# 1pathplanningzzj/pointnet_refine

Measured on AMD Instinct MI355X. Metric: lane segments/sec (fwd+bwd) at B=4096,N=1024; HBM GB/s vs roofline, higher is better.
Workload: dtype f32 (large GEMMs: 2xfp16-split MFMA, 3 products, fp32 accumulate); 1 GPU; LineRefineNet training step (fwd + deep-supervision L1 + bwd + Adam), B=4096/GPU, N=1024, M=32, C=4; global_batch=4096, points=1024, parallelism=dp1, decoder_chunk=4096

## Files before the change

### include/pointnet_refine_hip.h

```cpp
#ifndef POINTNET_REFINE_HIP_H
#define POINTNET_REFINE_HIP_H

#include <stddef.h>
#include <stdint.h>

#ifdef __cplusplus
extern "C" {
#endif

#define PRH_OK 0
#define PRH_ERR_ARG (-1)
#define PRH_ERR_WORKSPACE (-2)
#define PRH_ERR_HIP (-3)

#define PRH_MAX_LAYERS 8

typedef struct {
  const float* w;
  const float* b;
  const float* gamma;
  const float* beta;
  float* running_mean;
  float* running_var;
  int64_t* num_batches_tracked;
// ... 25 lines not shown
} prh_encoder_grads;

typedef struct {
  float* z_cat;
  float* z_fus;
  float* gate;
  float* bn_scale;
  float* bn_shift;
  float* bn_mean;
  float* bn_rstd;
  int32_t* argmax;
  float* op_amax;
} prh_encoder_saved;

size_t prh_encoder_workspace_bytes(int B, int N, int in_channel, int out_dim, int backward);

int prh_encoder_forward(const prh_encoder_params* prm, const float* ctx, int B, int N,
                        int training, float momentum, float eps,
                        float* fused, float* gfeat, const prh_encoder_saved* saved,
                        void* workspace, size_t workspace_bytes, int device, void* stream);

int prh_encoder_backward(const prh_encoder_params* prm, const float* ctx, int B, int N,
                         int training, float* d_fused, const float* d_gfeat, int d_fused_scratch,
                         const prh_encoder_saved* saved, const prh_encoder_grads* grads,
                         float* d_ctx, void* workspace, size_t workspace_bytes, int device,
                         void* stream);

typedef struct {
  uint16_t* z_cat;
  uint16_t* z_fus;
// ... 276 lines not shown
```

### pointnet_refine_amd/_lib.py

```python
from __future__ import annotations

import ctypes as C
import os
import subprocess
import threading

_HERE = os.path.dirname(os.path.abspath(__file__))
_ROOT = os.path.dirname(_HERE)
LIB_PATH = os.environ.get("PRH_LIB_PATH") or os.path.join(_HERE, "libpointnet_refine_hip.so")
_CSRC = os.path.join(_HERE, "csrc")
_SOURCES = [os.path.join(_CSRC, "prh_lib.hip")] + (sorted(
    os.path.join(_CSRC, f) for f in os.listdir(_CSRC) if f.endswith((".hpp", ".h", ".hip")) and f != "prh_lib.hip")
    if os.path.isdir(_CSRC) else [])
_HEADER = os.path.join(_ROOT, "include", "pointnet_refine_hip.h")

PRH_MAX_LAYERS = 8


class BnLayer(C.Structure):
    _fields_ = [("w", C.c_void_p), ("b", C.c_void_p), ("gamma", C.c_void_p), ("beta", C.c_void_p),
                ("running_mean", C.c_void_p), ("running_var", C.c_void_p),
                ("num_batches_tracked", C.c_void_p), ("cin", C.c_int), ("cout", C.c_int)]


# ... 13 lines not shown


class EncoderSaved(C.Structure):
    _fields_ = [("z_cat", C.c_void_p), ("z_fus", C.c_void_p), ("gate", C.c_void_p),
                ("bn_scale", C.c_void_p), ("bn_shift", C.c_void_p), ("bn_mean", C.c_void_p),
                ("bn_rstd", C.c_void_p), ("argmax", C.c_void_p), ("op_amax", C.c_void_p)]


class EncoderSavedBf16(C.Structure):
    _fields_ = [("z_cat", C.c_void_p), ("z_fus", C.c_void_p), ("gate", C.c_void_p),
                ("bn_scale", C.c_void_p), ("bn_shift", C.c_void_p), ("bn_mean", C.c_void_p),
                ("bn_rstd", C.c_void_p), ("argmax", C.c_void_p)]


EXPORTS = [
    "prh_encoder_workspace_bytes", "prh_encoder_forward", "prh_encoder_backward",
    "prh_encoder_bf16_workspace_bytes", "prh_encoder_forward_bf16", "prh_encoder_backward_bf16",
    "prh_linear_bf16_workspace_bytes", "prh_linear_forward_bf16", "prh_linear_backward_bf16",
    "prh_linear_forward_out16", "prh_linear_backward_dy16", "prh_attn_forward_kv16", "prh_attn_backward_kv16",
    "prh_encoder_fused_image_bytes", "prh_encoder_fused_prepare", "prh_encoder_fused_workspace_bytes",
    "prh_encoder_fused_forward",
    "prh_linear_forward_workspace_bytes", "prh_linear_forward", "prh_linear_forward_ex",
    "prh_linear_forward_full", "prh_operand_absmax_workspace_bytes", "prh_operand_absmax",
    "prh_linear_uses_operand_maxima", "prh_linear_backward_full", "prh_pos_hidden_forward", "prh_pos_hidden_backward_workspace_bytes",
    "prh_pos_hidden_backward", "prh_linear_small_forward", "prh_linear_small_backward_workspace_bytes",
    "prh_linear_small_backward",
    "prh_linear_backward_workspace_bytes", "prh_linear_backward", "prh_linear_backward_ex",
    "prh_mlp_stack_workspace_bytes", "prh_mlp_stack_forward", "prh_mlp_stack_backward",
    "prh_test_gemm_nt", "prh_test_gemm_tn_workspace_bytes", "prh_test_gemm_tn",
    "prh_test_gemm_tn_side_workspace_bytes", "prh_test_gemm_tn_side", "prh_test_xcc_map",
    "prh_profile_enable", "prh_profile_count", "prh_profile_reset", "prh_profile_read",
# ... 35 lines not shown
    hipcc = os.environ.get("HIPCC", "/opt/rocm/bin/hipcc")
    cmd = [hipcc, "--offload-arch=gfx950", "-O3", "-std=c++17", "-shared", "-fPIC",
           "-o", LIB_PATH, _SOURCES[0]]
    if verbose:
        print(" ".join(cmd))
    subprocess.run(cmd, check=True)
    return LIB_PATH


def _bind(lib):
    vp, i, f, sz, lg = C.c_void_p, C.c_int, C.c_float, C.c_size_t, C.c_long
    lib.prh_last_error.restype = C.c_char_p
    lib.prh_version.restype = C.c_char_p
    lib.prh_encoder_workspace_bytes.restype = sz
    lib.prh_encoder_workspace_bytes.argtypes = [i, i, i, i, i]
    lib.prh_encoder_forward.restype = i
    lib.prh_encoder_forward.argtypes = [C.POINTER(EncoderParams), vp, i, i, i, f, f, vp, vp,
                                        C.POINTER(EncoderSaved), vp, sz, i, vp]
    lib.prh_encoder_backward.restype = i
    lib.prh_encoder_backward.argtypes = [C.POINTER(EncoderParams), vp, i, i, i, vp, vp, i,
                                         C.POINTER(EncoderSaved), C.POINTER(EncoderGrads), vp, vp,
                                         sz, i, vp]
    lib.prh_encoder_bf16_workspace_bytes.restype = sz
    lib.prh_encoder_bf16_workspace_bytes.argtypes = [i, i, i, i, i]
    lib.prh_encoder_forward_bf16.restype = i
    lib.prh_encoder_forward_bf16.argtypes = [C.POINTER(EncoderParams), vp, i, i, i, f, f, vp, vp,
                                             C.POINTER(EncoderSavedBf16), vp, sz, i, vp]
    lib.prh_encoder_backward_bf16.restype = i
    lib.prh_encoder_backward_bf16.argtypes = [C.POINTER(EncoderParams), vp, i, i, i, vp, vp,
                                              C.POINTER(EncoderSavedBf16), C.POINTER(EncoderGrads), vp, vp,
# ... 229 lines not shown
```

### pointnet_refine_amd/csrc/prh_gemm_h2.hpp

```cpp
#pragma once
#include "prh_gemm_s3.hpp"

namespace prh {

constexpr int H2_BK = 32;
constexpr int H2_PLANE = 256 * H2_BK * 2;
constexpr int H2_OPER = 2 * H2_PLANE;
constexpr int H2_STAGE = 2 * H2_OPER;
constexpr int H2_LDS = 2 * H2_STAGE;

__device__ __forceinline__ int h2_off(int row, int k) {
  return row * 64 + ((((k >> 3) ^ (-(row >> 2))) & 3) << 4) + ((k & 7) << 1);
}

inline size_t h2_weight_bytes(int N, int K) {
  return S3_WHDR + (size_t)((N + 255) / 256) * ((K + H2_BK - 1) / H2_BK) * H2_OPER;
}

__global__ __launch_bounds__(256) void prep_weights_h2_kernel(const float* __restrict__ W, int N,
                                                              int K, long ldw, char* __restrict__ out,
                                                              const float* __restrict__ amax) {
  const int KT = (K + H2_BK - 1) / H2_BK;
  const int NT_ = (N + 255) / 256;
  const long total = (long)NT_ * 256 * KT * 4;
// ... 584 lines not shown
    __syncthreads();
    if (tid < 64) {
      float4 s = red[tid];
#pragma unroll
      for (int g = 1; g < 8; ++g) {
        const float4 t = red[tid + 64 * g];
        s.x += t.x; s.y += t.y; s.z += t.z; s.w += t.w;
      }
      const float inv = 1.f / sA;
      float* o = p.colsum + (size_t)split * p.Mo + m0 + c4;
      if (m0 + c4 + 3 < p.Mo) { o[0] = s.x * inv; o[1] = s.y * inv; o[2] = s.z * inv; o[3] = s.w * inv; }
    }
  }
}

}
```

### pointnet_refine_amd/csrc/prh_kernels.hpp

```cpp
#pragma once
#include <hip/hip_runtime.h>
#include <stdint.h>

namespace prh {

constexpr int BN_SLICES = 32;

__global__ __launch_bounds__(256) void bn_stage1_kernel(const float* __restrict__ ws_a,
                                                        const float* __restrict__ ws_b, int R,
                                                        long ld, int N, int tile_rows, int P,
                                                        int forward, double* __restrict__ out) {
  __shared__ double red[3][8][33];
  const int c = threadIdx.x & 31, g = threadIdx.x >> 5;
  const int col = blockIdx.x * 32 + c, sl = blockIdx.y;
  const int per = (R + BN_SLICES - 1) / BN_SLICES;
  const int r0 = sl * per, r1 = (r0 + per < R) ? r0 + per : R;
  const bool ok = col < N;
  double a = 0.0, b = 0.0, n = 0.0;
  if (ok)
    for (int i = r0 + g; i < r1; i += 8) {
      a += (double)ws_a[(size_t)i * ld + col];
      if (forward) {
        int ni = P - i * tile_rows;
        ni = ni > tile_rows ? tile_rows : (ni < 0 ? 0 : ni);
// ... 210 lines not shown
  int ix = 0;
  for (int t = 0; t < tiles_per_seg; ++t) {
    const size_t o = ((size_t)b * tiles_per_seg + t) * C + col;
    const float v = pmax[o];
    if (v > mx) { mx = v; ix = t * 128 + pidx[o]; }
    sum += psum[o];
  }
  gfeat[(size_t)b * 2 * C + col] = mx;
  gfeat[(size_t)b * 2 * C + C + col] = sum / (float)N;
  if (argmax != nullptr) argmax[(size_t)b * C + col] = ix;
}

__global__ __launch_bounds__(256) void combine_bwd_kernel(
    const float* dF, const float* __restrict__ d_gfeat, const int32_t* __restrict__ argmax,
    const float* __restrict__ zf, float* gate, const float* __restrict__ s,
    const float* __restrict__ t, int P, int N, int C, float* dy_out, float* ws_a, float* ws_b) {
  __shared__ float r1[4][64], r2[4][64];
  const int c = threadIdx.x & 63, g = threadIdx.x >> 6;
  const int col = blockIdx.y * 64 + c;
  const int row0 = blockIdx.x * 64 + g * 16;
  float s1 = 0.f, s2 = 0.f;
  if (col < C) {
    const float sc = s[col], sh = t[col];
    for (int i = 0; i < 16; ++i) {
      const int row = row0 + i;
      if (row >= P) break;
      const size_t off = (size_t)row * C + col;
      float d = dF != nullptr ? dF[off] : 0.f;
      if (d_gfeat != nullptr) {
        const int b = row / N, n = row - b * N;
        d += d_gfeat[(size_t)b * 2 * C + C + col] / (float)N;
        if (argmax[(size_t)b * C + col] == n) d += d_gfeat[(size_t)b * 2 * C + col];
      }
      const float z = zf[off], m = gate[off];
      const float pre = fmaf(z, sc, sh);
      const float r = fmaxf(pre, 0.f);
      const float sig = 2.f * m - 1.f;
      const float dy = pre > 0.f ? d * m : 0.f;
      gate[off] = d * r * 0.5f * sig * (1.f - sig);
      dy_out[off] = dy;
      s1 += dy;
      s2 = fmaf(dy, z, s2);
    }
  }
  r1[g][c] = s1; r2[g][c] = s2;
  __syncthreads();
  if (g == 0 && col < C) {
    for (int j = 1; j < 4; ++j) { s1 += r1[j][c]; s2 += r2[j][c]; }
    ws_a[(size_t)blockIdx.x * C + col] = s1;
    ws_b[(size_t)blockIdx.x * C + col] = s2;
  }
}

__global__ __launch_bounds__(256) void bn_apply_kernel(const float* __restrict__ z, long ldz,
                                                       const float* __restrict__ s,
                                                       const float* __restrict__ t, int P, int C,
                                                       int relu, float* y, long ldy) {
  const int col = blockIdx.y * 64 + (threadIdx.x & 63);
  const int row0 = blockIdx.x * 64 + (threadIdx.x >> 6) * 16;
  if (col >= C) return;
  const float sc = s[col], sh = t[col];
// ... 555 lines not shown
```

### pointnet_refine_amd/csrc/prh_lib.hip

```cpp
#include "../../include/pointnet_refine_hip.h"

#include <hip/hip_runtime.h>
#include <stdarg.h>
#include <stdio.h>
#include <string.h>

#include <mutex>
#include <vector>

#include <stdlib.h>

#include "prh_gemm.hpp"
#include "prh_attn.hpp"
#include "prh_attn16.hpp"
#include "prh_gemm_s3.hpp"
#include "prh_gemm_h2.hpp"
#include "prh_b16.hpp"
#include "prh_small.hpp"
#include "prh_attnfold.hpp"
#include "prh_fused.hpp"
#include "prh_context.hpp"
#include "prh_metrics.hpp"
#include "prh_drive.hpp"
#include "prh_match.hpp"
// ... 315 lines not shown
  if (n64 && (long)cdiv(p.M, 32) * cdiv(p.N, 64) >= 192) return launch_small_cfg<1, 2, 2, NN, EPI>(p, st);
  return launch_small_cfg<1, 1, 4, NN, EPI>(p, st);
}
constexpr int TN_SMALL_MAX_P = 16384;
inline bool small_tn_dims_ok(int P, int Mo, int Ni) {
  return P >= 64 && P <= TN_SMALL_MAX_P && (P & 63) == 0 && (Mo & 63) == 0 && (Ni & 63) == 0;
}
inline void small_tn_plan(int P, int Mo, int Ni, int& splits, int& rps) {
  const int tiles = (Mo / 64) * (Ni / 64), chunks = P / 64;
  int s = cdiv(512, tiles);
  s = s > chunks ? chunks : (s < 1 ? 1 : s);
  rps = cdiv(chunks, s) * 64;
  splits = cdiv(P, rps);
}

template <int PRO, int EPI>
int launch_nt(Cores c, NTParams& p, hipStream_t st, StatInfo* si = nullptr) {
  if (p.M <= 0 || p.N <= 0) return PRH_OK;
  if ((p.K & 3) || (PRO != PRO_GATE1 && (p.lda & 3)) || (p.ldw & 3) ||
      (PRO == PRO_BNBWD && (p.lda2 & 3)))
    return fail(PRH_ERR_ARG, "gemm_nt: K/lda/ldw must be multiples of 4 (K=%d lda=%ld ldw=%ld)",
                p.K, p.lda, p.ldw);
  if constexpr (PRO == PRO_NONE && EPI == EPI_BIAS) {
    if (c.mode == 4 && c.core == 2 && nt_b16_generic_ok(p)) return launch_nt_b16<PRO_NONE, EPI_BIAS, false, false>(p, st, si);
  }
  const bool want_pool = (p.flags & F_POOL) != 0;
  p.flags &= ~F_POOL;
  char nm[64];
  const double by = 4.0 * ((double)p.M * p.K * (PRO == PRO_BNBWD ? 2 : (PRO == PRO_GATE1 ? 0 : 1)) +
                           (double)p.M * p.N * (EPI == EPI_GATE ? 3 : (EPI == EPI_DGRAD ? 2 : 1)) +
                           (double)p.N * p.K);
  {
    if (p.wprep != nullptr && nt_use_s3(c, p.M, p.N, p.K) && p.lda <= 65536 && p.lda2 <= 65536 &&
        !(EPI == EPI_GATE && ((p.N | (int)p.ldc | (int)p.lde1 | (int)p.ldc2) & 3) != 0)) {
      const int KT = cdiv(p.K, S3_BK), NTl = cdiv(p.N, S3_BN);
      const long th = (long)NTl * 256 * KT * 2;
      float* hdr = reinterpret_cast<float*>(p.wprep);
      const char* img = p.wprep + S3_WHDR;
      if (c.core == 3) {
        if (p.amaxW == nullptr) {
          TRY_RC((measure_absmax<PRO_NONE>(p.W, p.ldw, nullptr, 0, nullptr, nullptr, nullptr, p.N, p.K, hdr, hdr + 64, st)));
          p.amaxW = hdr;
        }
        if (p.amaxA == nullptr) {
          TRY_RC((measure_absmax<PRO>(p.A, p.lda, p.A2, p.lda2, p.pa, p.pb, p.pc, p.M, p.K, hdr + 1, hdr + 64, st)));
          p.amaxA = hdr + 1;
// ... 81 lines not shown
    s = best;
  }
  const int minrows = pl.s3 ? 512 : 128;
  const int smax = cdiv(P, minrows) < 1 ? 1 : cdiv(P, minrows);
  if (s > smax) s = smax;
  if (s < 1) s = 1;
  int rps = cdiv(P, s);
  rps = cdiv(rps, bk) * bk;
  if (rps < bk) rps = bk;
  const int cap = (int)((2147483647L / (4L * (maxld < 4 ? 4 : maxld))) / bk * bk);
  if (pl.s3 && rps > cap) rps = cap;
  pl.splits = cdiv(P, rps) < 1 ? 1 : cdiv(P, rps);
  pl.rows_per_split = rps;
  return pl;
}
constexpr int TN_HDR = S3_HDR_FLOATS;
inline size_t tn_splits_bound(Cores cores, int P, int Mo, int Ni) {
  const size_t a = (size_t)tn_plan(cores, P, Mo, Ni, true).splits, b = (size_t)tn_plan(cores, P, Mo, Ni, false).splits;
  size_t c = (size_t)tn_plan(cores, P, Mo, Ni, true, 4).splits;
  if (small_tn_dims_ok(P, Mo, Ni)) {
    int ss, rr; small_tn_plan(P, Mo, Ni, ss, rr);
    if ((size_t)ss > c) c = (size_t)ss;
  }
  return a > b ? (a > c ? a : c) : (b > c ? b : c);
}
inline size_t tn_slab_floats(Cores c, int P, int Mo, int Ni) { return tn_splits_bound(c, P, Mo, Ni) * Mo * Ni + TN_HDR; }
inline size_t tn_colsum_floats(Cores c, int P, int Mo, int Ni) { return tn_splits_bound(c, P, Mo, Ni) * Mo; }

inline bool tn_side_ok(Cores c, const TNParams& p, const TNSide& s) {
  if (c.core != 3 || p.Mo <= 0 || p.Ni <= 0) return false;
  if (p.lda > TN_S3_MAX_LD || p.ldb > TN_S3_MAX_LD || p.lda2 > TN_S3_MAX_LD) return false;
  const TNPlan pl = tn_plan(c, p.P, p.Mo, p.Ni, true, p.lda > p.ldb ? p.lda : p.ldb);
  if (!pl.s3 || ((p.Mo | p.Ni | (int)p.lda | (int)p.ldb) & 3) != 0) return false;
  if ((long)pl.tiles_m * pl.tiles_n * pl.splits > ABSMAX_MAX_BLOCKS) return false;
// ... 1 lines not shown
         s.cols <= TR_SIDE_MAX_COLS && ((s.cols | (int)s.lddy | (int)s.ldz) & 3) == 0 && s.lddy <= 65536 &&
         s.ldz <= 65536 && al16(s.dy) && al16(s.z);
}

template <int PROA, int PROB>
int launch_tn(Cores c, TNParams& p, float* slab, float* colsum_slab, float* C, long ldc, float* colsum_out,
              hipStream_t st) {
  const bool side = p.side.dy != nullptr;
  if (side && !((PROA == PRO_NONE && (PROB == PRO_NONE || PROB == PRO_BNRELU)) && tn_side_ok(c, p, p.side)))
    return fail(PRH_ERR_ARG, "gemm_tn: this launch cannot carry a side job (Mo=%d Ni=%d P=%d)", p.Mo, p.Ni, p.P);
  if (p.Mo <= 0 || p.Ni <= 0) return PRH_OK;
  const bool ld_ok = p.lda <= TN_S3_MAX_LD && p.ldb <= TN_S3_MAX_LD && p.lda2 <= TN_S3_MAX_LD;
  long maxld = p.lda > p.ldb ? p.lda : p.ldb;
  if (PROA == PRO_BNBWD && p.lda2 > maxld) maxld = p.lda2;
  TNPlan pl = tn_plan(c, p.P, p.Mo, p.Ni, PROB != PRO_GATE1 && ld_ok, maxld);
  if (!pl.s3 && ((p.Mo & 3) || (p.Ni & 3) || (p.lda & 3) || (PROB != PRO_GATE1 && (p.ldb & 3))))
    return fail(PRH_ERR_ARG, "gemm_tn: Mo/Ni/lda/ldb must be multiples of 4 (Mo=%d Ni=%d)", p.Mo,
                p.Ni);
  p.tiles_m = pl.tiles_m; p.tiles_n = pl.tiles_n; p.splits = pl.splits;
  p.rows_per_split = pl.rows_per_split;
  p.slab = slab;
  p.colsum = colsum_out != nullptr ? colsum_slab : nullptr;
  const long blocks = (long)pl.tiles_m * pl.tiles_n * pl.splits;
  {
    char nm[64];
    const double by = 4.0 * ((double)p.P * p.Mo * (PROA == PRO_BNBWD ? 2 : 1) +
                             (double)p.P * (PROB == PRO_GATE1 ? 1 : p.Ni) + (double)p.Mo * p.Ni);
    bool done = false;
    if constexpr (PROB != PRO_GATE1) {
      if (pl.s3) {
        static const int attr_rc = allow_big_lds(gemm_tn_s3_kernel<PROA, PROB, 3>, gemm_tn_s3_kernel<PROA, PROB, 1>,
                                                 gemm_tn_s3_kernel<PROA, PROB, 2>);
        if (attr_rc != PRH_OK) return attr_rc;
        if (c.core == 3) {
          float* hdr = slab + (size_t)pl.splits * p.Mo * p.Ni;
          if (p.amaxA == nullptr) {
            TRY_RC((measure_absmax<PROA>(p.A, p.lda, p.A2, p.lda2, p.pa, p.pb, p.pc, p.P, p.Mo, hdr, hdr + 64, st)));
            p.amaxA = hdr;
          }
          if (p.amaxB == nullptr) {
            TRY_RC((measure_absmax<PROB>(p.B, p.ldb, nullptr, 0, p.qa, p.qb, nullptr, p.P, p.Ni, hdr + 1, hdr + 64, st)));
            p.amaxB = hdr + 1;
          }
// ... 381 lines not shown

struct LinearBwdWS { float* wT; float* slab; float* cslab; char* wprep; };
void linear_bwd_carve(Cores c, Arena& a, LinearBwdWS& w, int rows, int k, int n) {
  w.wprep = (char*)a.f(s3_weight_bytes(k, n) / sizeof(float) + 64);
  w.wT = a.f((size_t)k * n);
  w.slab = a.f(tn_slab_floats(c, rows, n, k));
  w.cslab = a.f(tn_colsum_floats(c, rows, n, k));
}
struct MlpWS { StackWS w; StackBwdScratch sc; float* dy_cat; };
void mlp_carve(Cores c, Arena& a, MlpWS& m, int P, const prh_bn_layer* ly, int L) {
  StackDims d = stack_dims(ly, L);
  stack_ws_carve(a, m.w, P, ly, L, max_cout(ly, L));
  stack_bwd_scratch_carve(c, a, m.sc, P, ly, L, 0, 0);
  m.dy_cat = a.f((size_t)P * d.off[L]);
}
struct EncWS { StackWS w; StackBwdScratch sc; float* fslab; float* fcslab; float* dy_cat; float* dyf; float* dU; float* gsum_a; float* gsum_b; };
void enc_carve(Cores c, Arena& a, EncWS& e, int P, const prh_bn_layer* conv, int cat, int od, int backward) {
  stack_ws_carve(a, e.w, P, conv, 5, cat > od ? cat : od, od, cat);
  if (!backward) return;
  stack_bwd_scratch_carve(c, a, e.sc, P, conv, 5, (size_t)od * cat, cat > od ? cat : od);
  const size_t fs = tn_slab_floats(c, P, od, cat), gs = tn_slab_floats(c, P, od, 64);
  const size_t fc = tn_colsum_floats(c, P, od, cat), gc = tn_colsum_floats(c, P, od, 64);
  e.fslab = a.f(fs > gs ? fs : gs);
  e.fcslab = a.f(fc > gc ? fc : gc);
  e.dy_cat = a.f((size_t)P * cat);
  e.dyf = backward == 2 ? nullptr : a.f((size_t)P * od);
  e.dU = a.f((size_t)P * 64);
  e.gsum_a = a.f(64);
  e.gsum_b = a.f(64);
}

typedef unsigned short u16;
struct Enc16WS {
  u16* xpad; float* w0pad; float* ws_a; float* ws_b; float* ws_c; double* stat2; char* wprep;
  float *ca, *cb, *cc, *wT, *slab, *cslab, *dU, *gsum_a, *gsum_b; u16 *dy_cat, *dyf;
  float* c1part;
};
constexpr int C1_WGRAD_BLOCKS = 1024;
inline bool conv_in_fp32_ok(int cin, int cout) { return cin <= 8 && cout == 64; }
inline int cin_pad8(int c) { return (c + 7) / 8 * 8; }
void enc16_carve(Arena& a, Enc16WS& e, int P, const int* ch , int cat, int od, bool backward) {
  const int c0p = cin_pad8(ch[0]);
  const int maxc = cat > od ? cat : od;
  e.xpad = (u16*)a.f(((size_t)P * c0p + 1) / 2);
// ... 397 lines not shown
  for (int l = 0; l < 5; ++l) c += prm->conv[l].cout;
  return c;
}

size_t prh_encoder_workspace_bytes(int B, int N, int in_channel, int out_dim, int backward) {
  const int P = B * N;
  prh_bn_layer ly[5];
  const int ch[6] = {in_channel, 64, 128, 256, 512, out_dim};
  for (int l = 0; l < 5; ++l) { ly[l].cin = ch[l]; ly[l].cout = ch[l + 1]; }
  const int cat = 64 + 128 + 256 + 512 + out_dim;
  Arena a; EncWS e;
  enc_carve(cores_of(gemm_mode()), a, e, P, ly, cat, out_dim, backward);
  return a.off + 256;
}

static int check_encoder(const prh_encoder_params* prm) {
  if (!prm) return fail(PRH_ERR_ARG, "encoder: null params");
  if (prm->in_channel < 4) return fail(PRH_ERR_ARG, "encoder: expected input to have at least 4 channels (x,y,z,intensity), got %d", prm->in_channel);
  if (prm->conv[0].cin != prm->in_channel) return fail(PRH_ERR_ARG, "encoder: conv1.cin != in_channel");
  TRY(check_stack(prm->conv, 5));
  if (prm->conv[4].cout != prm->out_dim) return fail(PRH_ERR_ARG, "encoder: conv5.cout != out_dim");
  if (prm->fusion.cin != enc_cat(prm) || prm->fusion.cout != prm->out_dim)
    return fail(PRH_ERR_ARG, "encoder: fusion layer shape mismatch");
  if (prm->out_dim % 4) return fail(PRH_ERR_ARG, "encoder: out_dim must be a multiple of 4");
  if (!prm->fusion.w || !prm->fusion.b || !prm->fusion.gamma || !prm->fusion.beta ||
      !prm->fusion.running_mean || !prm->fusion.running_var || !prm->gate_w1 || !prm->gate_b1 ||
      !prm->gate_w2 || !prm->gate_b2)
    return fail(PRH_ERR_ARG, "encoder: null parameter pointer");
  return PRH_OK;
}
// ... 87 lines not shown
    return fail(PRH_ERR_ARG, "encoder_backward: d_fused_scratch needs d_fused and no d_gfeat");
  enc_carve(c, a, ews, P, prm->conv, cat, od, d_fused_scratch ? 2 : 1);
  StackWS& w = ews.w;
  StackBwdScratch& sc = ews.sc;
  float *fslab = ews.fslab, *fcslab = ews.fcslab, *dy_cat = ews.dy_cat, *dU = ews.dU, *dyf = d_fused_scratch ? d_fused : ews.dyf;
  float *gsum_a = ews.gsum_a, *gsum_b = ews.gsum_b;
  if (!a.ok) return fail(PRH_ERR_WORKSPACE, "encoder_backward: workspace too small (%zu bytes)", workspace_bytes);
  StackDims d = stack_dims(prm->conv, 5);
  if (d.cin0p != d.cin0) {
    TRY(copy_cols(ctx, d.cin0, d.cin0, w.xpad, d.cin0p, d.cin0p, (size_t)P, st));
    TRY(copy_cols(prm->conv[0].w, d.cin0, d.cin0, w.w0pad, d.cin0p, d.cin0p, (size_t)prm->conv[0].cout, st));
  }

  hipLaunchKernelGGL(combine_bwd_kernel, dim3(cdiv(P, 64), cdiv(od, 64)), dim3(256), 0, st, d_fused,
                     d_gfeat, sv->argmax, sv->z_fus, sv->gate, sv->bn_scale + cat,
                     sv->bn_shift + cat, P, N, od, dyf, w.ws_a, w.ws_b);
  LAUNCH_CHECK();
  hipLaunchKernelGGL(bn_stage1_kernel, dim3(cdiv(od, 32), BN_SLICES), dim3(256), 0, st, w.ws_a, w.ws_b,
                     cdiv(P, 64), (long)od, od, 64, P, 0, w.stat2);
  LAUNCH_CHECK();
  hipLaunchKernelGGL(bn_bwd_finalize_kernel, dim3(cdiv(od, 128)), dim3(128), 0, st, w.stat2, P, od,
                     prm->fusion.gamma, sv->bn_mean + cat, sv->bn_rstd + cat,
                     training, sc.ca, sc.cb, sc.cc, gr->fusion.dgamma, gr->fusion.dbeta,
                     gr->fusion.db);
  LAUNCH_CHECK();
  float* dG = sv->gate;

  StatInfo si5;
  const float* dzf_amax = nullptr;
  const bool matf = dz_in_place(c, od, (long)od, (long)od);
  if (matf) {
    TRY(materialize_dz(dyf, (long)od, sv->z_fus, (long)od, sc.ca, sc.cb, sc.cc, P, od, sc.hdr[0], st));
// ... 25 lines not shown
    p.ws_a = w.ws_a; p.ws_b = w.ws_b;
    p.flags = F_MASK | F_STATS;
    if (matf) TRY((launch_nt<PRO_NONE, EPI_DGRAD>(c, p, st, &si5)));
    else TRY((launch_nt<PRO_BNBWD, EPI_DGRAD>(c, p, st, &si5)));
    si5.ld = cat; si5.off = d.off[4];
  }
  float* dx = d_ctx;
  TRY(stack_backward(c, prm->conv, 5, ctx, P, training, dy_cat, (long)cat, sv->z_cat, (long)cat,
                     sv->bn_scale, sv->bn_shift, sv->bn_mean, sv->bn_rstd, gr->conv, dx, w, sc, si5,
                     st, sv->op_amax, &hf));

  {
    TNParams t; memset(&t, 0, sizeof(t));
    t.A = dG; t.lda = od; t.B = ctx + 3; t.ldb = C; t.qa = prm->gate_w1; t.qb = prm->gate_b1;
    t.P = P; t.Mo = od; t.Ni = 64;
    TRY((launch_tn<PRO_NONE, PRO_GATE1>(c, t, fslab, fcslab, gr->d_gate_w2, 64L, gr->d_gate_b2, st)));
    TRY(transpose(prm->gate_w2, od, 64, sc.wT, st));
    NTParams p; memset(&p, 0, sizeof(p));
    p.A = dG; p.lda = od; p.W = sc.wT; p.ldw = od; p.M = P; p.N = 64; p.K = od;
    p.C = dU; p.ldc = 64; p.E1 = ctx + 3; p.lde1 = C; p.es = prm->gate_w1; p.et = prm->gate_b1;
    p.ws_a = w.ws_a; p.ws_b = w.ws_b;
    p.flags = F_MASK | F_STATS | F_E1_ROWVEC;
    StatInfo sig;
    TRY((launch_nt<PRO_NONE, EPI_DGRAD>(c, p, st, &sig)));
    hipLaunchKernelGGL(partials_reduce_kernel, dim3(2), dim3(1024), 0, st, w.ws_a, w.ws_b,
                       sig.count, 64, gr->d_gate_b1 ? gr->d_gate_b1 : gsum_a,
                       gr->d_gate_w1 ? gr->d_gate_w1 : gsum_b);
    LAUNCH_CHECK();
    if (d_ctx != nullptr) {
      hipLaunchKernelGGL(gate1_dctx_kernel, dim3(cdiv(P, 4)), dim3(256), 0, st, dU, P, 64,
                         prm->gate_w1, d_ctx, (long)C);
      LAUNCH_CHECK();
    }
  }
  return PRH_OK;
}

// ... 1419 lines not shown
```

Before: 9612 segments/s.

## Add narrow-N split-fp16 GEMM kernels for gate backward with fused dG absmax

```diff
diff --git a/include/pointnet_refine_hip.h b/include/pointnet_refine_hip.h
--- a/include/pointnet_refine_hip.h
+++ b/include/pointnet_refine_hip.h
@@ -63,6 +63,8 @@
 } prh_encoder_saved;
 
 size_t prh_encoder_workspace_bytes(int B, int N, int in_channel, int out_dim, int backward);
+
+size_t prh_encoder_backward_ws_offset(int B, int N, int in_channel, int out_dim, int backward, int which);
 
 int prh_encoder_forward(const prh_encoder_params* prm, const float* ctx, int B, int N,
                         int training, float momentum, float eps,
diff --git a/pointnet_refine_amd/_lib.py b/pointnet_refine_amd/_lib.py
--- a/pointnet_refine_amd/_lib.py
+++ b/pointnet_refine_amd/_lib.py
@@ -51,7 +51,7 @@
 
 
 EXPORTS = [
-    "prh_encoder_workspace_bytes", "prh_encoder_forward", "prh_encoder_backward",
+    "prh_encoder_workspace_bytes", "prh_encoder_backward_ws_offset", "prh_encoder_forward", "prh_encoder_backward",
     "prh_encoder_bf16_workspace_bytes", "prh_encoder_forward_bf16", "prh_encoder_backward_bf16",
     "prh_linear_bf16_workspace_bytes", "prh_linear_forward_bf16", "prh_linear_backward_bf16",
     "prh_linear_forward_out16", "prh_linear_backward_dy16", "prh_attn_forward_kv16", "prh_attn_backward_kv16",
@@ -117,6 +117,8 @@
     lib.prh_version.restype = C.c_char_p
     lib.prh_encoder_workspace_bytes.restype = sz
     lib.prh_encoder_workspace_bytes.argtypes = [i, i, i, i, i]
+    lib.prh_encoder_backward_ws_offset.restype = sz
+    lib.prh_encoder_backward_ws_offset.argtypes = [i, i, i, i, i, i]
     lib.prh_encoder_forward.restype = i
     lib.prh_encoder_forward.argtypes = [C.POINTER(EncoderParams), vp, i, i, i, f, f, vp, vp,
                                         C.POINTER(EncoderSaved), vp, sz, i, vp]
diff --git a/pointnet_refine_amd/csrc/prh_gemm_h2.hpp b/pointnet_refine_amd/csrc/prh_gemm_h2.hpp
--- a/pointnet_refine_amd/csrc/prh_gemm_h2.hpp
+++ b/pointnet_refine_amd/csrc/prh_gemm_h2.hpp
@@ -622,4 +622,241 @@
   }
 }
 
-}
+constexpr int H2N_WPLANE = 64 * H2_BK * 2;
+constexpr int H2N_STAGE = H2_OPER + 2 * H2N_WPLANE;
+constexpr int H2N_LDS = 2 * H2N_STAGE;
+static_assert(8 * 32 * EPI_LDW * 4 <= H2N_LDS, "epilogue scratch must fit in the stage buffers");
+
+template <int EPI>
+__global__ __launch_bounds__(512, 4) void gemm_nt_h2n_kernel(const NTParams p, const char* __restrict__ Wp) {
+  extern __shared__ __attribute__((aligned(16))) char smem[];
+  const int tid = threadIdx.x, lane = tid & 63, wave = tid >> 6;
+  const int l15 = lane & 15, kc = lane >> 4;
+  const int wm = wave * 32;
+  const int tile_m = blockIdx.x, m0 = tile_m * 256;
+  const int KT = (p.K + H2_BK - 1) / H2_BK;
+  const int sc = (tid & 7) * 4;
+  const int sr = tid >> 3;
+  const float sA = pow2_scale(load_amax(p.amaxA));
+  const float unscale = 1.f / (sA * pow2_scale(load_amax(p.amaxW)));
+
+  f32x4 acc[2][4];
+#pragma unroll
+  for (int i = 0; i < 2; ++i)
+#pragma unroll
+    for (int j = 0; j < 4; ++j)
+#pragma unroll
+      for (int r = 0; r < 4; ++r) acc[i][j][r] = 0.f;
+
+  int arows = p.M - m0; arows = arows > 256 ? 256 : arows;
+  const __amdgpu_buffer_rsrc_t rsA = __builtin_amdgcn_make_buffer_rsrc(
+      (void*)(p.A + (size_t)m0 * p.lda), 0, (int)(((size_t)(arows - 1) * p.lda + p.K) * 4), 0x00020000);
+  int voA[4];
+#pragma unroll
+  for (int j = 0; j < 4; ++j) voA[j] = ((sr + 64 * j) * (int)p.lda + sc) * 4;
+  const char* wsrc = Wp + (tid < 256 ? tid * 16 : H2_PLANE + (tid - 256) * 16);
+  float4 ra[2][5];
+  auto load_tile = [&](int kt, float4 (&r)[5]) {
+    const int so = kt * (H2_BK * 4);
+#pragma unroll
+    for (int j = 0; j < 4; ++j)
+      r[j] = __builtin_bit_cast(float4, __builtin_amdgcn_raw_buffer_load_b128(rsA, voA[j] + so, 0, 0));
+    r[4] = *reinterpret_cast<const float4*>(wsrc + (size_t)kt * H2_OPER);
+  };
+  auto store_tile = [&](int kt, char* st, const float4 (&r_)[5]) {
+    const bool kok = kt * H2_BK + sc < p.K;
+#pragma unroll
+    for (int j = 0; j < 4; ++j) {
+      float4 v = r_[j];
+      v.x = kok ? v.x * sA : 0.f; v.y = kok ? v.y * sA : 0.f; v.z = kok ? v.z * sA : 0.f; v.w = kok ? v.w * sA : 0.f;
+      uint2 h, l;
+      split2h(v.x, v.y, h.x, l.x);
+      split2h(v.z, v.w, h.y, l.y);
+      char* q = st + h2_off(sr + 64 * j, sc);
+      *reinterpret_cast<uint2*>(q) = h;
+      *reinterpret_cast<uint2*>(q + H2_PLANE) = l;
+    }
+    *reinterpret_cast<float4*>(st + H2_OPER + tid * 16) = r_[4];
+  };
+  auto compute = [&](const char* st) {
+    f16x8 ah[2], al[2];
+#pragma unroll
+    for (int i = 0; i < 2; ++i) {
+      const char* q = st + h2_off(wm + i * 16 + l15, kc * 8);
+      ah[i] = *reinterpret_cast<const f16x8*>(q);
+      al[i] = *reinterpret_cast<const f16x8*>(q + H2_PLANE);
+    }
+#pragma unroll
+    for (int j = 0; j < 4; ++j) {
+      const char* q = st + H2_OPER + h2_off(j * 16 + l15, kc * 8);
+      const f16x8 wh = *reinterpret_cast<const f16x8*>(q);
+      const f16x8 wl = *reinterpret_cast<const f16x8*>(q + H2N_WPLANE);
+#pragma unroll
+      for (int i = 0; i < 2; ++i) {
+        acc[i][j] = __builtin_amdgcn_mfma_f32_16x16x32_f16(al[i], wh, acc[i][j], 0, 0, 0);
+        acc[i][j] = __builtin_amdgcn_mfma_f32_16x16x32_f16(ah[i], wl, acc[i][j], 0, 0, 0);
+        acc[i][j] = __builtin_amdgcn_mfma_f32_16x16x32_f16(ah[i], wh, acc[i][j], 0, 0, 0);
+      }
+    }
+  };
+  auto iter = [&](int kt, auto cs) {
+    constexpr int CS = decltype(cs)::value;
+    if (kt + 2 < KT) load_tile(kt + 2, ra[CS ^ 1]);
+    compute(smem + (kt & 1) * H2N_STAGE);
+    if (kt + 1 < KT) store_tile(kt + 1, smem + ((kt + 1) & 1) * H2N_STAGE, ra[CS]);
+    __syncthreads();
+  };
+  load_tile(0, ra[0]);
+  if (KT > 1) load_tile(1, ra[1]);
+  store_tile(0, smem, ra[0]);
+  __syncthreads();
+  for (int kt = 0; kt < KT; kt += 2) {
+    iter(kt, std::integral_constant<int, 1>{});
+    if (kt + 1 < KT) iter(kt + 1, std::integral_constant<int, 0>{});
+  }
+#pragma unroll
+  for (int i = 0; i < 2; ++i)
+#pragma unroll
+    for (int j = 0; j < 4; ++j)
+#pragma unroll
+      for (int r = 0; r < 4; ++r) acc[i][j][r] *= unscale;
+  nt_epilogue_vec<EPI, 1>(acc, p, m0 + wm, 0, tile_m * 8 + wave, lane,
+                          reinterpret_cast<float*>(smem) + wave * (32 * EPI_LDW));
+}
+
+__global__ __launch_bounds__(512, 2) void gemm_tn_trn_kernel(const TNParams p) {
+  extern __shared__ __attribute__((aligned(16))) char smem[];
+  const int tid = threadIdx.x, lane = tid & 63, wave = tid >> 6;
+  const int wm = wave * 32;
+  int b = xcd_remap(blockIdx.x, gridDim.x);
+  const int tile_m = b % p.tiles_m;
+  const int split = b / p.tiles_m;
+  const int m0 = tile_m * 256;
+  const int p_begin = split * p.rows_per_split;
+  int p_end = p_begin + p.rows_per_split;
+  if (p_end > p.P) p_end = p.P;
+  const int nrows = p_end - p_begin > 0 ? p_end - p_begin : 0;
+  const int KT = (nrows + S3_BK - 1) / S3_BK;
+
+  const int c4 = lane * 4, r8 = wave;
+  const bool aok = (m0 + c4) < p.Mo, bok = lane < 16 && c4 < p.Ni;
+  const float sA = pow2_scale(load_amax(p.amaxA)), sB = pow2_scale(load_amax(p.amaxB));
+  const float sAm = aok ? sA : 0.f;
+  float4 qa = zero4(), qb = zero4();
+  if (bok) {
+    qa = ldg4(p.qa + c4); qb = ldg4(p.qb + c4);
+    qa.x *= sB; qa.y *= sB; qa.z *= sB; qa.w *= sB; qb.x *= sB; qb.y *= sB; qb.z *= sB; qb.w *= sB;
+  }
+  const bool want_cs = p.colsum != nullptr;
+
+  f32x16 acc[2];
+#pragma unroll
+  for (int j = 0; j < 2; ++j)
+#pragma unroll
+    for (int r = 0; r < 16; ++r) acc[j][r] = 0.f;
+
+  int acols = p.Mo - m0; acols = acols > 256 ? 256 : acols;
+  const size_t abytes = nrows > 0 ? ((size_t)(nrows - 1) * p.lda + acols) * 4 : 0;
+  const size_t bbytes = nrows > 0 ? ((size_t)(nrows - 1) * p.ldb + 1) * 4 : 0;
+  const __amdgpu_buffer_rsrc_t rsA = __builtin_amdgcn_make_buffer_rsrc(
+      (void*)(p.A + (size_t)p_begin * p.lda + m0), 0, (int)abytes, 0x00020000);
+  const __amdgpu_buffer_rsrc_t rsB = __builtin_amdgcn_make_buffer_rsrc(
+      (void*)(p.B + (size_t)p_begin * p.ldb), 0, (int)bbytes, 0x00020000);
+  const int stepA = (int)p.lda * 4, stepB = (int)p.ldb * 4;
+  const int voA = r8 * stepA + c4 * 4, voB = r8 * stepB;
+
+  float4 va[2][2];
+  float vi[2][2];
+  float4 cs = zero4();
+  auto load_tile = [&](int kt, float4 (&xa)[2], float (&xi)[2]) {
+    const int oa = voA + kt * S3_BK * stepA, ob = voB + kt * S3_BK * stepB;
+#pragma unroll
+    for (int j = 0; j < 2; ++j) {
+      xa[j] = __builtin_bit_cast(float4, __builtin_amdgcn_raw_buffer_load_b128(rsA, oa + j * 8 * stepA, 0, 0));
+      xi[j] = __builtin_bit_cast(float, __builtin_amdgcn_raw_buffer_load_b32(rsB, ob + j * 8 * stepB, 0, 0));
+    }
+  };
+  auto store_tile = [&](char* st, const float4 (&xa)[2], const float (&xi)[2]) {
+#pragma unroll
+    for (int j = 0; j < 2; ++j) {
+      float4 a = xa[j];
+      a.x *= sAm; a.y *= sAm; a.z *= sAm; a.w *= sAm;
+      if (want_cs) { cs.x += a.x; cs.y += a.y; cs.z += a.z; cs.w += a.w; }
+      uint2 h, l;
+      char* q = st + (r8 + 8 * j) * TR_ROW + c4 * 2;
+      split2h(a.x, a.y, h.x, l.x);
+      split2h(a.z, a.w, h.y, l.y);
+      *reinterpret_cast<uint2*>(q) = h;
+      *reinterpret_cast<uint2*>(q + TR_PLANE) = l;
+      if (lane < 16) {
+        const float4 y = pro_apply<PRO_GATE1>(make_float4(xi[j], 0.f, 0.f, 0.f), zero4(), qa, qb, zero4());
+        split2h(y.x, y.y, h.x, l.x);
+        split2h(y.z, y.w, h.y, l.y);
+        *reinterpret_cast<uint2*>(q + TR_OPER) = h;
+        *reinterpret_cast<uint2*>(q + TR_OPER + TR_PLANE) = l;
+      }
+    }
+  };
+  auto compute = [&](const char* st) {
+    const f16x8 ah = tr_fragment(st, wm, lane);
+    const f16x8 al = tr_fragment(st + TR_PLANE, wm, lane);
+#pragma unroll
+    for (int j = 0; j < 2; ++j) {
+      const f16x8 wh = tr_fragment(st + TR_OPER, j * 32, lane);
+      const f16x8 wl = tr_fragment(st + TR_OPER + TR_PLANE, j * 32, lane);
+      acc[j] = __builtin_amdgcn_mfma_f32_32x32x16_f16(al, wh, acc[j], 0, 0, 0);
+      acc[j] = __builtin_amdgcn_mfma_f32_32x32x16_f16(ah, wl, acc[j], 0, 0, 0);
+      acc[j] = __builtin_amdgcn_mfma_f32_32x32x16_f16(ah, wh, acc[j], 0, 0, 0);
+    }
+  };
+  if (KT > 0) {
+    load_tile(0, va[0], vi[0]);
+    load_tile(1, va[1], vi[1]);
+    store_tile(smem, va[0], vi[0]);
+  }
+  __syncthreads();
+  auto iter = [&](int kt, auto cs_) {
+    constexpr int CS = decltype(cs_)::value;
+    load_tile(kt + 2, va[CS ^ 1], vi[CS ^ 1]);
+    compute(smem + (kt & 1) * TR_STAGE);
+    store_tile(smem + ((kt + 1) & 1) * TR_STAGE, va[CS], vi[CS]);
+    __syncthreads();
+  };
+  int kt = 0;
+  for (; kt + 1 < KT; kt += 2) {
+    iter(kt, std::integral_constant<int, 1>{});
+    iter(kt + 1, std::integral_constant<int, 0>{});
+  }
+  if (kt < KT) iter(kt, std::integral_constant<int, 1>{});
+
+  const float unscale = 1.f / (sA * sB);
+  const int half = lane >> 5, l31 = lane & 31;
+  float* out = p.slab + (size_t)split * p.Mo * p.Ni;
+#pragma unroll
+  for (int nt = 0; nt < 2; ++nt) {
+    const int col = nt * 32 + l31;
+#pragma unroll
+    for (int r = 0; r < 16; ++r) {
+      const int row = m0 + wm + crow(r, half);
+      if (row < p.Mo && col < p.Ni) out[(size_t)row * p.Ni + col] = acc[nt][r] * unscale;
+    }
+  }
+  if (want_cs) {
+    float4* red = reinterpret_cast<float4*>(smem);
+    red[tid] = cs;
+    __syncthreads();
+    if (tid < 64) {
+      float4 s = red[tid];
+#pragma unroll
+      for (int g = 1; g < 8; ++g) {
+        const float4 t = red[tid + 64 * g];
+        s.x += t.x; s.y += t.y; s.z += t.z; s.w += t.w;
+      }
+      const float inv = 1.f / sA;
+      float* o = p.colsum + (size_t)split * p.Mo + m0 + c4;
+      if (m0 + c4 + 3 < p.Mo) { o[0] = s.x * inv; o[1] = s.y * inv; o[2] = s.z * inv; o[3] = s.w * inv; }
+    }
+  }
+}
+
+}
diff --git a/pointnet_refine_amd/csrc/prh_kernels.hpp b/pointnet_refine_amd/csrc/prh_kernels.hpp
--- a/pointnet_refine_amd/csrc/prh_kernels.hpp
+++ b/pointnet_refine_amd/csrc/prh_kernels.hpp
@@ -248,12 +248,13 @@
 __global__ __launch_bounds__(256) void combine_bwd_kernel(
     const float* dF, const float* __restrict__ d_gfeat, const int32_t* __restrict__ argmax,
     const float* __restrict__ zf, float* gate, const float* __restrict__ s,
-    const float* __restrict__ t, int P, int N, int C, float* dy_out, float* ws_a, float* ws_b) {
-  __shared__ float r1[4][64], r2[4][64];
+    const float* __restrict__ t, int P, int N, int C, float* dy_out, float* ws_a, float* ws_b,
+    float* __restrict__ dg_part) {
+  __shared__ float r1[4][64], r2[4][64], r3[4];
   const int c = threadIdx.x & 63, g = threadIdx.x >> 6;
   const int col = blockIdx.y * 64 + c;
   const int row0 = blockIdx.x * 64 + g * 16;
-  float s1 = 0.f, s2 = 0.f;
+  float s1 = 0.f, s2 = 0.f, gm = 0.f;
   if (col < C) {
     const float sc = s[col], sh = t[col];
     for (int i = 0; i < 16; ++i) {
@@ -271,14 +272,23 @@
       const float r = fmaxf(pre, 0.f);
       const float sig = 2.f * m - 1.f;
       const float dy = pre > 0.f ? d * m : 0.f;
-      gate[off] = d * r * 0.5f * sig * (1.f - sig);
+      const float dg = d * r * 0.5f * sig * (1.f - sig);
+      gate[off] = dg;
+      gm = fmaxf(gm, fabsf(dg));
       dy_out[off] = dy;
       s1 += dy;
       s2 = fmaf(dy, z, s2);
     }
   }
   r1[g][c] = s1; r2[g][c] = s2;
-  __syncthreads();
+  if (dg_part != nullptr) {
+#pragma unroll
+    for (int o = 32; o > 0; o >>= 1) gm = fmaxf(gm, __shfl_xor(gm, o));
+    if (c == 0) r3[g] = gm;
+  }
+  __syncthreads();
+  if (dg_part != nullptr && threadIdx.x == 0)
+    dg_part[(size_t)blockIdx.x * gridDim.y + blockIdx.y] = fmaxf(fmaxf(r3[0], r3[1]), fmaxf(r3[2], r3[3]));
   if (g == 0 && col < C) {
     for (int j = 1; j < 4; ++j) { s1 += r1[j][c]; s2 += r2[j][c]; }
     ws_a[(size_t)blockIdx.x * C + col] = s1;
diff --git a/pointnet_refine_amd/csrc/prh_lib.hip b/pointnet_refine_amd/csrc/prh_lib.hip
--- a/pointnet_refine_amd/csrc/prh_lib.hip
+++ b/pointnet_refine_amd/csrc/prh_lib.hip
@@ -353,6 +353,18 @@
   splits = cdiv(P, rps);
 }
 
+constexpr int NARROW_MIN_ROWS = 64, NARROW_MIN_K = 256;
+inline bool nt_narrow_ok(Cores c, const NTParams& p) {
+  return c.core == 3 && p.wprep != nullptr && p.N >= 4 && p.N <= 64 && p.K >= NARROW_MIN_K && p.K <= 8192 &&
+         p.M >= NARROW_MIN_ROWS && ((p.N | (int)p.ldc | p.K | (int)p.lda | (int)p.ldw) & 3) == 0 && p.lda <= 65536 &&
+         al16(p.A) && al16(p.C) && p.C2 == nullptr &&
+         (p.E1 == nullptr || (p.flags & F_E1_ROWVEC) != 0 || ((int)p.lde1 & 3) == 0);
+}
+inline bool tn_narrow_ok(Cores c, const TNParams& p) {
+  return c.core == 3 && p.Ni >= 4 && p.Ni <= 64 && p.Mo >= NARROW_MIN_K && p.P >= NARROW_MIN_ROWS &&
+         ((p.Mo | p.Ni | (int)p.lda) & 3) == 0 && p.lda <= 4096 && p.ldb <= 4096 && al16(p.A) && p.side.dy == nullptr;
+}
+
 template <int PRO, int EPI>
 int launch_nt(Cores c, NTParams& p, hipStream_t st, StatInfo* si = nullptr) {
   if (p.M <= 0 || p.N <= 0) return PRH_OK;
@@ -369,6 +381,33 @@
   const double by = 4.0 * ((double)p.M * p.K * (PRO == PRO_BNBWD ? 2 : (PRO == PRO_GATE1 ? 0 : 1)) +
                            (double)p.M * p.N * (EPI == EPI_GATE ? 3 : (EPI == EPI_DGRAD ? 2 : 1)) +
                            (double)p.N * p.K);
+  if constexpr (PRO == PRO_NONE && EPI == EPI_DGRAD) {
+    if (nt_narrow_ok(c, p)) {
+      float* hdr = reinterpret_cast<float*>(p.wprep);
+      if (p.amaxW == nullptr) {
+        TRY_RC((measure_absmax<PRO_NONE>(p.W, p.ldw, nullptr, 0, nullptr, nullptr, nullptr, p.N, p.K, hdr, hdr + 64, st)));
+        p.amaxW = hdr;
+      }
+      if (p.amaxA == nullptr) {
+        TRY_RC((measure_absmax<PRO_NONE>(p.A, p.lda, nullptr, 0, nullptr, nullptr, nullptr, p.M, p.K, hdr + 1, hdr + 64, st)));
+        p.amaxA = hdr + 1;
+      }
+      const int KT2 = cdiv(p.K, H2_BK);
+      hipLaunchKernelGGL(prep_weights_h2_kernel, dim3((unsigned)cdiv(256L * KT2 * 4, 256)), dim3(256), 0, st, p.W,
+                         p.N, p.K, p.ldw, p.wprep + S3_WHDR, p.amaxW);
+      LAUNCH_CHECK();
+      p.tiles_n = 1;
+      static const int attr_h2n = allow_big_lds(gemm_nt_h2n_kernel<EPI>);
+      if (attr_h2n != PRH_OK) return attr_h2n;
+      snprintf(nm, sizeof(nm), "gemm_nt_h2n<%d,%d> K=%d N=%d", PRO, EPI, p.K, p.N);
+      ProfScope ps(nm, 2.0 * p.M * (double)p.N * p.K, by, st);
+      hipLaunchKernelGGL((gemm_nt_h2n_kernel<EPI>), dim3((unsigned)cdiv(p.M, 256)), dim3(512), H2N_LDS, st, p,
+                         (const char*)(p.wprep + S3_WHDR));
+      LAUNCH_CHECK();
+      if (si) { si->count = 8 * cdiv(p.M, 256); si->rows = 32; }
+      return PRH_OK;
+    }
+  }
   {
     if (p.wprep != nullptr && nt_use_s3(c, p.M, p.N, p.K) && p.lda <= 65536 && p.lda2 <= 65536 &&
         !(EPI == EPI_GATE && ((p.N | (int)p.ldc | (int)p.lde1 | (int)p.ldc2) & 3) != 0)) {
@@ -480,10 +519,30 @@
   pl.rows_per_split = rps;
   return pl;
 }
+inline TNPlan tn_plan_narrow(int P, int Mo, long maxld = TN_S3_MAX_LD) {
+  TNPlan pl;
+  pl.s3 = true;
+  pl.tiles_m = cdiv(Mo, 256);
+  pl.tiles_n = 1;
+  int s = cdiv(512, pl.tiles_m);
+  const int smax = cdiv(P, 512) < 1 ? 1 : cdiv(P, 512);
+  s = s > smax ? smax : (s < 1 ? 1 : s);
+  int rps = cdiv(cdiv(P, s), S3_BK) * S3_BK;
+  if (rps < S3_BK) rps = S3_BK;
+  const int cap = (int)((2147483647L / (4L * (maxld < 4 ? 4 : maxld))) / S3_BK * S3_BK);
+  if (rps > cap) rps = cap;
+  pl.splits = cdiv(P, rps) < 1 ? 1 : cdiv(P, rps);
+  pl.rows_per_split = rps;
+  return pl;
+}
 constexpr int TN_HDR = S3_HDR_FLOATS;
 inline size_t tn_splits_bound(Cores cores, int P, int Mo, int Ni) {
   const size_t a = (size_t)tn_plan(cores, P, Mo, Ni, true).splits, b = (size_t)tn_plan(cores, P, Mo, Ni, false).splits;
   size_t c = (size_t)tn_plan(cores, P, Mo, Ni, true, 4).splits;
+  if (cores.core == 3 && Ni <= 64 && Mo >= NARROW_MIN_K) {
+    const size_t n1 = (size_t)tn_plan_narrow(P, Mo, 4).splits, n2 = (size_t)tn_plan_narrow(P, Mo).splits;
+    c = n1 > c ? n1 : c; c = n2 > c ? n2 : c;
+  }
   if (small_tn_dims_ok(P, Mo, Ni)) {
     int ss, rr; small_tn_plan(P, Mo, Ni, ss, rr);
     if ((size_t)ss > c) c = (size_t)ss;
@@ -515,6 +574,11 @@
   long maxld = p.lda > p.ldb ? p.lda : p.ldb;
   if (PROA == PRO_BNBWD && p.lda2 > maxld) maxld = p.lda2;
   TNPlan pl = tn_plan(c, p.P, p.Mo, p.Ni, PROB != PRO_GATE1 && ld_ok, maxld);
+  bool narrow = false;
+  if constexpr (PROA == PRO_NONE && PROB == PRO_GATE1) {
+    narrow = tn_narrow_ok(c, p);
+    if (narrow) pl = tn_plan_narrow(p.P, p.Mo, maxld);
+  }
   if (!pl.s3 && ((p.Mo & 3) || (p.Ni & 3) || (p.lda & 3) || (PROB != PRO_GATE1 && (p.ldb & 3))))
     return fail(PRH_ERR_ARG, "gemm_tn: Mo/Ni/lda/ldb must be multiples of 4 (Mo=%d Ni=%d)", p.Mo,
                 p.Ni);
@@ -528,6 +592,26 @@
     const double by = 4.0 * ((double)p.P * p.Mo * (PROA == PRO_BNBWD ? 2 : 1) +
                              (double)p.P * (PROB == PRO_GATE1 ? 1 : p.Ni) + (double)p.Mo * p.Ni);
     bool done = false;
+    if constexpr (PROA == PRO_NONE && PROB == PRO_GATE1) {
+      if (narrow) {
+        static const int attr_trn = allow_big_lds(gemm_tn_trn_kernel);
+        if (attr_trn != PRH_OK) return attr_trn;
+        float* hdr = slab + (size_t)pl.splits * p.Mo * p.Ni;
+        if (p.amaxA == nullptr) {
+          TRY_RC((measure_absmax<PRO_NONE>(p.A, p.lda, nullptr, 0, nullptr, nullptr, nullptr, p.P, p.Mo, hdr, hdr + 64, st)));
+          p.amaxA = hdr;
+        }
+        if (p.amaxB == nullptr) {
+          TRY_RC((measure_absmax<PRO_GATE1>(p.B, p.ldb, nullptr, 0, p.qa, p.qb, nullptr, p.P, p.Ni, hdr + 1, hdr + 64, st)));
+          p.amaxB = hdr + 1;
+        }
+        p.pace = nullptr;
+        snprintf(nm, sizeof(nm), "gemm_tn_h2trn<%d,%d> Mo=%d Ni=%d", PROA, PROB, p.Mo, p.Ni);
+        ProfScope ps(nm, 2.0 * p.P * (double)p.Mo * p.Ni, by, st);
+        hipLaunchKernelGGL(gemm_tn_trn_kernel, dim3((unsigned)blocks), dim3(512), TR_LDS, st, p);
+        done = true;
+      }
+    }
     if constexpr (PROB != PRO_GATE1) {
       if (pl.s3) {
         static const int attr_rc = allow_big_lds(gemm_tn_s3_kernel<PROA, PROB, 3>, gemm_tn_s3_kernel<PROA, PROB, 1>,
@@ -939,9 +1023,12 @@
   stack_bwd_scratch_carve(c, a, m.sc, P, ly, L, 0, 0);
   m.dy_cat = a.f((size_t)P * d.off[L]);
 }
-struct EncWS { StackWS w; StackBwdScratch sc; float* fslab; float* fcslab; float* dy_cat; float* dyf; float* dU; float* gsum_a; float* gsum_b; };
+struct EncWS { StackWS w; StackBwdScratch sc; float* fslab; float* fcslab; float* dy_cat; float* dyf; float* dU; float* gsum_a; float* gsum_b;
+               char* gwprep; float* dgpart; size_t gwprep_off, dU_off; };
+constexpr int ENC_DG_AMAX = 2;
 void enc_carve(Cores c, Arena& a, EncWS& e, int P, const prh_bn_layer* conv, int cat, int od, int backward) {
   stack_ws_carve(a, e.w, P, conv, 5, cat > od ? cat : od, od, cat);
+  e.gwprep = nullptr; e.dgpart = nullptr; e.gwprep_off = e.dU_off = (size_t)-1;
   if (!backward) return;
   stack_bwd_scratch_carve(c, a, e.sc, P, conv, 5, (size_t)od * cat, cat > od ? cat : od);
   const size_t fs = tn_slab_floats(c, P, od, cat), gs = tn_slab_floats(c, P, od, 64);
@@ -950,9 +1037,18 @@
   e.fcslab = a.f(fc > gc ? fc : gc);
   e.dy_cat = a.f((size_t)P * cat);
   e.dyf = backward == 2 ? nullptr : a.f((size_t)P * od);
+  a.off = align_up(a.off, 256);
+  e.dU_off = a.off;
   e.dU = a.f((size_t)P * 64);
   e.gsum_a = a.f(64);
   e.gsum_b = a.f(64);
+  e.gwprep = nullptr; e.dgpart = nullptr; e.gwprep_off = (size_t)-1;
+  if (c.core == 3) {
+    a.off = align_up(a.off, 256);
+    e.gwprep_off = a.off;
+    e.gwprep = (char*)a.f(h2_weight_bytes(64, od) / sizeof(float) + 64);
+    e.dgpart = a.f((size_t)cdiv(P, 64) * cdiv(od, 64));
+  }
 }
 
 typedef unsigned short u16;
@@ -1380,6 +1476,17 @@
   return a.off + 256;
 }
 
+size_t prh_encoder_backward_ws_offset(int B, int N, int in_channel, int out_dim, int backward, int which) {
+  prh_bn_layer ly[5];
+  const int ch[6] = {in_channel, 64, 128, 256, 512, out_dim};
+  for (int l = 0; l < 5; ++l) { ly[l].cin = ch[l]; ly[l].cout = ch[l + 1]; }
+  Arena a; EncWS e;
+  enc_carve(cores_of(gemm_mode()), a, e, B * N, ly, 64 + 128 + 256 + 512 + out_dim, out_dim, backward);
+  if (!backward) return (size_t)-1;
+  if (which == 1) return e.dU_off;
+  return e.gwprep_off == (size_t)-1 ? (size_t)-1 : e.gwprep_off + ENC_DG_AMAX * sizeof(float);
+}
+
 static int check_encoder(const prh_encoder_params* prm) {
   if (!prm) return fail(PRH_ERR_ARG, "encoder: null params");
   if (prm->in_channel < 4) return fail(PRH_ERR_ARG, "encoder: expected input to have at least 4 channels (x,y,z,intensity), got %d", prm->in_channel);
@@ -1497,8 +1604,15 @@
 
   hipLaunchKernelGGL(combine_bwd_kernel, dim3(cdiv(P, 64), cdiv(od, 64)), dim3(256), 0, st, d_fused,
                      d_gfeat, sv->argmax, sv->z_fus, sv->gate, sv->bn_scale + cat,
-                     sv->bn_shift + cat, P, N, od, dyf, w.ws_a, w.ws_b);
-  LAUNCH_CHECK();
+                     sv->bn_shift + cat, P, N, od, dyf, w.ws_a, w.ws_b, ews.dgpart);
+  LAUNCH_CHECK();
+  const float* dg_amax = nullptr;
+  if (ews.dgpart != nullptr) {
+    float* hdr = reinterpret_cast<float*>(ews.gwprep);
+    TRY((measure_absmax<PRO_NONE>(ews.dgpart, (long)cdiv(od, 64), nullptr, 0, nullptr, nullptr, nullptr, (long)cdiv(P, 64),
+                                  cdiv(od, 64), hdr + ENC_DG_AMAX, hdr + 64, st)));
+    dg_amax = hdr + ENC_DG_AMAX;
+  }
   hipLaunchKernelGGL(bn_stage1_kernel, dim3(cdiv(od, 32), BN_SLICES), dim3(256), 0, st, w.ws_a, w.ws_b,
                      cdiv(P, 64), (long)od, od, 64, P, 0, w.stat2);
   LAUNCH_CHECK();
@@ -1554,6 +1668,7 @@
     TNParams t; memset(&t, 0, sizeof(t));
     t.A = dG; t.lda = od; t.B = ctx + 3; t.ldb = C; t.qa = prm->gate_w1; t.qb = prm->gate_b1;
     t.P = P; t.Mo = od; t.Ni = 64;
+    t.amaxA = dg_amax;
     TRY((launch_tn<PRO_NONE, PRO_GATE1>(c, t, fslab, fcslab, gr->d_gate_w2, 64L, gr->d_gate_b2, st)));
     TRY(transpose(prm->gate_w2, od, 64, sc.wT, st));
     NTParams p; memset(&p, 0, sizeof(p));
@@ -1561,6 +1676,7 @@
     p.C = dU; p.ldc = 64; p.E1 = ctx + 3; p.lde1 = C; p.es = prm->gate_w1; p.et = prm->gate_b1;
     p.ws_a = w.ws_a; p.ws_b = w.ws_b;
     p.flags = F_MASK | F_STATS | F_E1_ROWVEC;
+    p.wprep = ews.gwprep; p.amaxA = dg_amax;
     StatInfo sig;
     TRY((launch_nt<PRO_NONE, EPI_DGRAD>(c, p, st, &sig)));
     hipLaunchKernelGGL(partials_reduce_kernel, dim3(2), dim3(1024), 0, st, w.ws_a, w.ws_b,
```

After: 9657 segments/s, median of 5. About the same (+0.5%).
